# jhidalgocarrio/slam-localization

Hardware: NVIDIA B200
Metric: filter-steps/sec (predict+update) (higher is better)
Workload: dtype f64

## Files before the change

slam-localization_b200/csrc/slb_usckf.cu:

```cuda
#include <cstdlib>

#include "slb_predict12.cuh"
#include "slb_usckf_step.cuh"

namespace slbd {

__global__ void usckf_clone_kernel(slb::FilterArgs a, int mode) {
    const int64_t t = (int64_t)blockIdx.x * blockDim.x + threadIdx.x;
    const int per = 13 + 12 * 12 * 2;
    if (t >= (int64_t)a.B * per) return;
    const int inst = (int)(t / per), e = (int)(t - (int64_t)inst * per);
    double *P = a.P + (size_t)inst * a.pstride, *mu = a.mu + (size_t)inst * a.qstride;
    auto sym = [&](int r, int c) { return r >= c ? P[tri(r, c)] : P[tri(c, r)]; };
    if (e < 13) {
        if (mode == SLB_STATEK_I) mu[13 + e] = mu[26 + e];
        else mu[e] = mu[13 + e];
        return;
    }
    const int q = e - 13, blk = q / 144, rc = q - blk * 144, r = rc / 12, c = rc - r * 12;
    if (mode == SLB_STATEK_I) {
        if (blk == 0) {
            const double v = sym(24 + r, 24 + c);
            if (c <= r) P[tri(12 + r, 12 + c)] = v;
            P[tri(24 + r, 12 + c)] = v;
        } else {
            P[tri(24 + r, c)] = 0.0;
            P[tri(12 + r, c)] = 0.0;
        }
    } else if (blk == 0) {
        const double v = sym(12 + r, 12 + c);
        if (c <= r) P[tri(r, c)] = v;
        P[tri(12 + r, c)] = v;
    }
}

__global__ void usckf_set_measurement_kernel(slb::FilterArgs a, int mode) {
    const int N = 36 + a.nk + a.nl, NP = N * (N + 1) / 2;
    const int nfe = NP - 666;
    const int per = nfe + (mode == SLB_STATEK ? a.nk : a.nl);
    const int64_t t = (int64_t)blockIdx.x * blockDim.x + threadIdx.x;
    if (t >= (int64_t)a.B * per) return;
    const int inst = (int)(t / per), e = (int)(t - (int64_t)inst * per);
    double *P = a.P + (size_t)inst * a.pstride, *mu = a.mu + (size_t)inst * a.qstride;
    const int len = mode == SLB_STATEK ? a.nk : a.nl;
    const int f0 = mode == SLB_STATEK ? 0 : a.nk;
    if (e >= nfe) {
        const int c = e - nfe;
        mu[39 + f0 + c] = a.z[(size_t)inst * len + c];
        return;
    }
    int r = 36;
    while (tri(r + 1, 0) - 666 <= e) ++r;
    const int c = e - (tri(r, 0) - 666);
    const int fr = r - 36, fc = c - 36;
    double v = 0.0;
    if (c >= 36) {
        const bool rin = fr >= f0 && fr < f0 + len, cin = fc >= f0 && fc < f0 + len;
        if (rin && cin) v = a.R[(fr - f0) * len + (fc - f0)];
        else if (!rin && !cin) v = P[tri(r, c)];
    }
    P[tri(r, c)] = v;
}

}

namespace slb {

template <int PM>
static int launch_predict_t(const FilterArgs &a, cudaStream_t s) {
    constexpr int WPB = 8;
    constexpr size_t smem = (size_t)WPB * slbd::PRED_SM * sizeof(double);
    auto kern = slbd::predict12_kernel<PM, WPB, 24, 26, true>;
    SLB_CUDA(cudaFuncSetAttribute(kern, cudaFuncAttributeMaxDynamicSharedMemorySize, (int)smem));
    kern<<<(a.B + WPB - 1) / WPB, WPB * 32, smem, s>>>(a);
    count_launch();
    SLB_CUDA(cudaGetLastError());
    return SLB_OK;
}

#define SLB_USCKF_SHAPES(X) X(3, 0) X(3, 3) X(3, 6) X(3, 9) X(6, 0) X(6, 3) X(6, 6) X(9, 0) X(9, 3)
bool usckf_shape_supported(int nk, int nl) {
#define SLB_USCKF_SHAPE(NK_, NL_) \
    if (nk == NK_ && nl == NL_) return true;
    SLB_USCKF_SHAPES(SLB_USCKF_SHAPE)
#undef SLB_USCKF_SHAPE
    return false;
}

template <int NK, int NL, bool PRED, bool UPD>
static int launch_step_t(const FilterArgs &a, cudaStream_t s) {
    typedef slbd::StepCfg<NK, NL> C;
    constexpr size_t pw = (size_t)C::SM * sizeof(double);
    constexpr size_t SM_BYTES = 228 * 1024, CTA_MAX = 227 * 1024, RSV = 1024;
#ifdef SLB_USCKF_WPB
    constexpr int WPB = SLB_USCKF_WPB;
#else
    constexpr int WPB = 2 * (6 * pw + RSV) <= SM_BYTES ? 6 : 4;
#endif
    constexpr size_t smem = (size_t)WPB * pw;
    constexpr int fit = (int)(SM_BYTES / (smem + RSV));
    constexpr int cap = 12 / WPB < 1 ? 1 : 12 / WPB;
    constexpr int MINB = fit > cap ? cap : fit < 1 ? 1 : fit;
    auto kern = slbd::usckf_step_kernel<SLB_PM_USCKF_TEST, NK, NL, PRED, UPD, WPB, MINB>;
    SLB_CUDA(cudaFuncSetAttribute(kern, cudaFuncAttributeMaxDynamicSharedMemorySize, (int)smem));
    static const int ahead = [] {
        const char *e = getenv("SLB_USCKF_PREFETCH");
        int dev = 0, sms = 148;
        cudaGetDevice(&dev);
        cudaDeviceGetAttribute(&sms, cudaDevAttrMultiProcessorCount, dev);
        return (e ? atoi(e) : 0) * sms * WPB * MINB;
    }();
    FilterArgs b = a;
    b.prefetch = ahead;
    static const size_t pad = [] {
        const char *e = getenv("SLB_USCKF_CTAS");
        const int n = e ? atoi(e) : 0;
        return n == 1 ? (size_t)(200 * 1024) - smem : n == 2 ? (size_t)(110 * 1024) - smem : (size_t)0;
    }();
    if (pad) SLB_CUDA(cudaFuncSetAttribute(kern, cudaFuncAttributeMaxDynamicSharedMemorySize, (int)(smem + pad)));
    kern<<<(a.B + WPB - 1) / WPB, WPB * 32, smem + pad, s>>>(b);
    count_launch();
    SLB_CUDA(cudaGetLastError());
    return SLB_OK;
}

template <int NK, int NL>
static int launch_step_nknl(bool predict, const FilterArgs &a, cudaStream_t s) {
    return predict ? launch_step_t<NK, NL, true, true>(a, s) : launch_step_t<NK, NL, false, true>(a, s);
}

int launch_usckf(int pm, int mm, bool predict, bool update, const FilterArgs &a, cudaStream_t s) {
    if (predict && pm != SLB_PM_USCKF_TEST) return set_error(SLB_ERR_INVALID, "usckf: unsupported process model");
    if (update && mm != SLB_MM_USCKF_VO) return set_error(SLB_ERR_INVALID, "usckf: unsupported measurement model");
    if (predict && !update) return launch_predict_t<SLB_PM_USCKF_TEST>(a, s);
    if (update) {
#define SLB_USCKF_SHAPE(NK_, NL_) \
    if (a.nk == NK_ && a.nl == NL_) return launch_step_nknl<NK_, NL_>(predict, a, s);
        SLB_USCKF_SHAPES(SLB_USCKF_SHAPE)
#undef SLB_USCKF_SHAPE
        return set_error(SLB_ERR_INVALID, "usckf update: (nk, nl) is not one of the built shapes (see slb_usckf_shape_supported)");
    }
    return SLB_OK;
}

int launch_usckf_clone(int mode, const FilterArgs &a, cudaStream_t s) {
    if (mode != SLB_STATEK_I && mode != SLB_STATEK_L) return SLB_OK;
    const int64_t work = (int64_t)a.B * (13 + 288);
    slbd::usckf_clone_kernel<<<(unsigned)((work + 255) / 256), 256, 0, s>>>(a, mode);
    count_launch();
    SLB_CUDA(cudaGetLastError());
    return SLB_OK;
}

int launch_usckf_set_measurement(int mode, const FilterArgs &a, cudaStream_t s) {
    if (mode != SLB_STATEK && mode != SLB_STATEK_L) return SLB_OK;
    const int N = 36 + a.nk + a.nl;
    const int len = mode == SLB_STATEK ? a.nk : a.nl;
    if (len == 0) return SLB_OK;
    const int64_t work = (int64_t)a.B * (N * (N + 1) / 2 - 666 + len);
    slbd::usckf_set_measurement_kernel<<<(unsigned)((work + 255) / 256), 256, 0, s>>>(a, mode);
    count_launch();
    SLB_CUDA(cudaGetLastError());
    return SLB_OK;
}

}
```

slam-localization_b200/csrc/slb_usckf_step.cuh:

```cuda
#pragma once
#include "slb_predict12.cuh"

#ifndef SLB_USCKF_CTA_SYNC
#define SLB_USCKF_CTA_SYNC 0
#endif
#if SLB_USCKF_CTA_SYNC
#define SLB_CTA_SYNC() __syncthreads()
#else
#define SLB_CTA_SYNC() ((void)0)
#endif

namespace slbd {

template <int NK_, int NL_>
struct StepCfg {
    static constexpr int NK = NK_, NL = NL_, NF = NK_ + NL_;
    static constexpr int N = 36 + NK_ + NL_;
    static constexpr int NP = N * (N + 1) / 2;
    static constexpr int PSTR = (NP + 15) / 16 * 16;
    static constexpr int QD = 39 + NK_ + NL_;
    static constexpr int QS = (QD + 1) / 2 * 2;
    static constexpr int NT = (N + 7) / 8;
    static constexpr int NPAD = 8 * NT;
    static constexpr int JM = 36 + NK_;
    static constexpr int NPAN = (JM + 3) / 4;
    static constexpr int NCOL = 4 * NPAN;
    static constexpr int JLAST = (NCOL - 1) >> 3;
    static constexpr int NGRP = (NPAN + 3) / 4;
    static constexpr int PL = 2 * NPAD + 8;
    static constexpr int PS4 = 2 * PL + 2;
    static constexpr int KP = (NK_ + 3) / 4 * 4;
    static constexpr int LF = 4 * PS4;
    static constexpr int LRAW = 2 * PL;
    static constexpr int KK = 2 * NPAD * KP + NPAD;
    static constexpr int SCR0 = (LF + LRAW > KK ? LF + LRAW : KK);
    static constexpr int WGS = 16 * NK_;
    static constexpr int UPD_SCR = SCR0 + WGS + NPAD;
    static constexpr int PRED_SCR = PRED_LS + 28 * PRED_DS + 144 + 12 * PRED_DS + 16 + 16;
    static constexpr int SCR = (UPD_SCR > PRED_SCR ? UPD_SCR : PRED_SCR);
    static constexpr int ZS = (NK_ + 1) / 2 * 2;
    static constexpr int SM = PSTR + QS + SCR + ZS + 2;
    static_assert(NK_ % 3 == 0 && NK_ >= 3, "the VO model moves 3-D features");
    static_assert(N <= 64, "two rows per lane");
    static_assert(SM % 2 == 0 && PSTR % 2 == 0 && QS % 2 == 0, "16-byte alignment of the bulk copies");
};

SLB_DEV void bulk_s2g(void *gdst, const void *ssrc, unsigned bytes) {
    asm volatile("cp.async.bulk.global.shared::cta.bulk_group [%0], [%1], %2;\n cp.async.bulk.commit_group;\n" ::"l"(gdst),
                 "r"(saddr(ssrc)), "r"(bytes)
                 : "memory");
}
SLB_DEV void bulk_prefetch_l2(const void *gsrc, unsigned bytes) {
    asm volatile("cp.async.bulk.prefetch.L2.global [%0], %1;\n" ::"l"(gsrc), "r"(bytes) : "memory");
}
SLB_DEV void bulk_store_wait() { asm volatile("cp.async.bulk.wait_group.read 0;\n" ::: "memory"); }
SLB_DEV void fence_proxy_async() { asm volatile("fence.proxy.async.shared::cta;\n" ::: "memory"); }

template <int M>
SLB_DEV bool sym_inverse(const double *S, double *Si) {
    double L[M * (M + 1) / 2], dd[M], rd[M];
    bool ok = true;
#pragma unroll
    for (int k = 0; k < M; ++k) {
        double d = S[tri(k, k)];
#pragma unroll
        for (int p = 0; p < k; ++p) d = fma(-L[tri(k, p)] * L[tri(k, p)], dd[p], d);
        ok = ok && (d > 0.0);
        dd[k] = d;
        rd[k] = rcp_fast(d);
#pragma unroll
        for (int i = k + 1; i < M; ++i) {
            double s = S[tri(i, k)];
#pragma unroll
            for (int p = 0; p < k; ++p) s = fma(-L[tri(i, p)] * L[tri(k, p)], dd[p], s);
            L[tri(i, k)] = s * rd[k];
        }
    }
    double X[M * (M + 1) / 2];
#pragma unroll
    for (int j = 0; j < M; ++j) {
        X[tri(j, j)] = 1.0;
#pragma unroll
        for (int i = j + 1; i < M; ++i) {
            double s = 0.0;
#pragma unroll
            for (int p = j; p < i; ++p) s = fma(-L[tri(i, p)], X[tri(p, j)], s);
            X[tri(i, j)] = s;
        }
    }
#pragma unroll
    for (int i = 0; i < M; ++i)
#pragma unroll
        for (int j = 0; j <= i; ++j) {
            double s = 0.0;
#pragma unroll
            for (int k = i; k < M; ++k) s = fma(X[tri(k, i)] * rd[k], X[tri(k, j)], s);
            Si[tri(i, j)] = s;
        }
    return ok;
}

template <int NK>
SLB_DEV void vo_model(const double *pk, const double *qk, const double *pi, const double *qi, const double *f, double *z) {
    double dq[4];
    quat_cmul(qi, qk, dq);
#pragma unroll
    for (int c = 0; c < NK; c += 3) {
        double rz[3];
        rotmat_apply(dq, f + c, rz);
        z[c] = rz[0] + (pk[0] - pi[0]);
        z[c + 1] = rz[1] + (pk[1] - pi[1]);
        z[c + 2] = rz[2] + (pk[2] - pi[2]);
    }
}

SLB_DEV void warp_sum12(const double *v, double *out, double *slots, int lane) {
    double a[8], b[4], c[2], d1;
    const bool h16 = lane & 16, h8 = lane & 8, h4 = lane & 4, h2 = lane & 2;
#pragma unroll
    for (int i = 0; i < 8; ++i) {
        const double lo = v[i], hi = i < 4 ? v[8 + i] : 0.0;
        const double r = __shfl_xor_sync(FULL, h16 ? lo : hi, 16);
        a[i] = (h16 ? hi : lo) + r;
    }
#pragma unroll
    for (int i = 0; i < 4; ++i) {
        const double r = __shfl_xor_sync(FULL, h8 ? a[i] : a[4 + i], 8);
        b[i] = (h8 ? a[4 + i] : a[i]) + r;
    }
#pragma unroll
    for (int i = 0; i < 2; ++i) {
        const double r = __shfl_xor_sync(FULL, h4 ? b[i] : b[2 + i], 4);
        c[i] = (h4 ? b[2 + i] : b[i]) + r;
    }
    {
        const double r = __shfl_xor_sync(FULL, h2 ? c[0] : c[1], 2);
        d1 = (h2 ? c[1] : c[0]) + r;
    }
    d1 += __shfl_xor_sync(FULL, d1, 1);
    const int idx = (h16 ? 8 : 0) + (h8 ? 4 : 0) + (h4 ? 2 : 0) + (h2 ? 1 : 0);
    __syncwarp();
    if (!(lane & 1)) slots[idx] = d1;
    __syncwarp();
#pragma unroll
    for (int i = 0; i < 6; ++i) {
        const double2 t = *reinterpret_cast<const double2 *>(slots + 2 * i);
        out[2 * i] = t.x;
        out[2 * i + 1] = t.y;
    }
}

template <class C>
struct UpdState {
    double c0[C::NT][C::JLAST + 1], c1[C::NT][C::JLAST + 1];
    double px0[C::NK], px1[C::NK];
    double esum[C::NK], eep[C::NK * (C::NK + 1) / 2];
    double z0[C::NK];
    bool ok;
};

template <class C, int G>
SLB_DEV void sigma_group(UpdState<C> &s, const double *mus_, const double *Lf, double *Wg, const double *dv, int lane) {
    constexpr int NK = C::NK, PS4 = C::PS4;
    double mus[40 + NK];
    {
        const double2 *m2 = reinterpret_cast<const double2 *>(mus_);
#pragma unroll
        for (int e = 0; e < 4; ++e) { const double2 v = m2[e]; mus[2 * e] = v.x; mus[2 * e + 1] = v.y; }
#pragma unroll
        for (int e = 13; e < 17; ++e) { const double2 v = m2[e]; mus[2 * e] = v.x; mus[2 * e + 1] = v.y; }
#pragma unroll
        for (int c = 0; c < NK; ++c) mus[39 + c] = mus_[39 + c];
    }
    constexpr int col0 = 16 * G;
    constexpr int ncols = C::NCOL - col0 < 16 ? C::NCOL - col0 : 16;
    const bool neg = lane & 1, act = (lane >> 1) < ncols;
    const int jl = act ? lane >> 1 : 0;
    const double rs = rsqrt_fast(dv[col0 + jl]);
    const double sgn = act ? (neg ? -rs : rs) : 0.0;
    const double *col = Lf + (jl >> 2) * PS4 + ((jl & 3) >> 1) * C::PL + (jl & 1);
    auto Lc = [&](int r) -> double { return sgn * col[2 * r]; };
    double xpk[3], xqk[4], xpi[3], xqi[4], xf[NK];
    if (col0 <= 5) {
#pragma unroll
        for (int c = 0; c < 3; ++c) xpk[c] = mus[c] + Lc(c);
        const double v[3] = {Lc(3), Lc(4), Lc(5)};
        const double q[4] = {mus[3], mus[4], mus[5], mus[6]};
        double e[4];
        so3_exp(v, 1.0, e);
        quat_mul(q, e, xqk);
    } else {
#pragma unroll
        for (int c = 0; c < 3; ++c) xpk[c] = mus[c];
#pragma unroll
        for (int c = 0; c < 4; ++c) xqk[c] = mus[3 + c];
    }
    if (col0 <= 29) {
#pragma unroll
        for (int c = 0; c < 3; ++c) xpi[c] = mus[26 + c] + Lc(24 + c);
        const double v[3] = {Lc(27), Lc(28), Lc(29)};
        const double q[4] = {mus[29], mus[30], mus[31], mus[32]};
        double e[4];
        so3_exp(v, 1.0, e);
        quat_mul(q, e, xqi);
    } else {
#pragma unroll
        for (int c = 0; c < 3; ++c) xpi[c] = mus[26 + c];
#pragma unroll
        for (int c = 0; c < 4; ++c) xqi[c] = mus[29 + c];
    }
#pragma unroll
    for (int c = 0; c < NK; ++c) xf[c] = mus[39 + c] + Lc(36 + c);
    double z[NK];
    vo_model<NK>(xpk, xqk, xpi, xqi, xf, z);
    double e[NK];
#pragma unroll
    for (int c = 0; c < NK; ++c) {
        e[c] = act ? z[c] - s.z0[c] : 0.0;
        s.esum[c] += e[c];
        const double zp = __shfl_xor_sync(FULL, z[c], 1);
        if (act && !neg) Wg[c * 16 + jl] = (0.5 * rs) * (z[c] - zp);
    }
#pragma unroll
    for (int r = 0; r < NK; ++r)
#pragma unroll
        for (int c = 0; c <= r; ++c) s.eep[tri(r, c)] = fma(e[r], e[c], s.eep[tri(r, c)]);
    __syncwarp();
    const bool has1 = lane + 32 < C::NPAD;
#pragma unroll
    for (int qq = 0; qq < ncols / 4; ++qq) {
        const double *pa = Lf + qq * PS4 + 2 * lane, *pb = pa + C::PL;
        const double2 x01 = *reinterpret_cast<const double2 *>(pa), x23 = *reinterpret_cast<const double2 *>(pb);
        double2 y01 = make_double2(0.0, 0.0), y23 = y01;
        if (has1) { y01 = *reinterpret_cast<const double2 *>(pa + 64); y23 = *reinterpret_cast<const double2 *>(pb + 64); }
#pragma unroll
        for (int c = 0; c < NK; ++c) {
            const double2 w01 = *reinterpret_cast<const double2 *>(Wg + c * 16 + 4 * qq);
            const double2 w23 = *reinterpret_cast<const double2 *>(Wg + c * 16 + 4 * qq + 2);
            s.px0[c] = fma(x23.y, w23.y, fma(x23.x, w23.x, fma(x01.y, w01.y, fma(x01.x, w01.x, s.px0[c]))));
            s.px1[c] = fma(y23.y, w23.y, fma(y23.x, w23.x, fma(y01.y, w01.y, fma(y01.x, w01.x, s.px1[c]))));
        }
    }
}

template <class C, int P>
struct PanelStep {
    SLB_DEV static void run(UpdState<C> &s, const double *mus, double *Lf, double *Lraw, double *Wg, double *dv, int lane) {
        constexpr int NT = C::NT, JLAST = C::JLAST, PS4 = C::PS4;
        constexpr int K = 4 * P, J0 = K >> 3, H = (K >> 2) & 1, Q = P & 3;
        constexpr int I1 = (K + 4) >> 3;
        const int a_ = lane & 3, b_ = lane >> 2;
        double *Lq = Lf + Q * PS4;
        constexpr int PL = C::PL;
        if ((a_ >> 1) == H) {
#pragma unroll
            for (int I = J0; I < NT; ++I)
                *reinterpret_cast<double2 *>(Lraw + (a_ & 1) * PL + 2 * (8 * I + b_)) = make_double2(s.c0[I][J0], s.c1[I][J0]);
        }
        __syncwarp();
        double m10, m20, m30, m21, m31, m32, r0, r1, r2, r3, d0, d1, d2, d3;
        {
            const double *A = Lraw + 2 * K, *Bp = A + PL;
            const double a00 = A[0];
            const double2 a1 = *reinterpret_cast<const double2 *>(A + 2);
            const double2 a2 = *reinterpret_cast<const double2 *>(A + 4);
            const double a22 = Bp[4];
            const double2 a3 = *reinterpret_cast<const double2 *>(A + 6), a3b = *reinterpret_cast<const double2 *>(Bp + 6);
            d0 = a00;
            r0 = rcp_fast(d0);
            m10 = a1.x * r0; m20 = a2.x * r0; m30 = a3.x * r0;
            d1 = fma(-a1.x, m10, a1.y);
            const double u21 = fma(-a2.x, m10, a2.y), u31 = fma(-a3.x, m10, a3.y);
            r1 = rcp_fast(d1);
            m21 = u21 * r1; m31 = u31 * r1;
            d2 = fma(-u21, m21, fma(-a2.x, m20, a22));
            const double u32 = fma(-u31, m21, fma(-a3.x, m20, a3b.x));
            r2 = rcp_fast(d2);
            m32 = u32 * r2;
            d3 = fma(-u32, m32, fma(-u31, m31, fma(-a3.x, m30, a3b.y)));
            r3 = rcp_fast(d3);
            s.ok = s.ok && (d0 > 0.0) && (d1 > 0.0) && (d2 > 0.0) && (d3 > 0.0);
        }
        if (lane == 0) {
            *reinterpret_cast<double2 *>(dv + K) = make_double2(d0, d1);
            *reinterpret_cast<double2 *>(dv + K + 2) = make_double2(d2, d3);
        }
        auto finish = [&](int i, bool have) {
            const double2 x01 = *reinterpret_cast<const double2 *>(Lraw + 2 * i);
            const double2 x23 = *reinterpret_cast<const double2 *>(Lraw + PL + 2 * i);
            const double u0 = x01.x;
            const double u1 = fma(-u0, m10, x01.y);
            const double u2 = fma(-u1, m21, fma(-u0, m20, x23.x));
            const double u3 = fma(-u2, m32, fma(-u1, m31, fma(-u0, m30, x23.y)));
            double2 u01, u23;
            u01.x = i >= K ? u0 : 0.0;
            u01.y = i >= K + 1 ? u1 : 0.0;
            u23.x = i >= K + 2 ? u2 : 0.0;
            u23.y = i >= K + 3 ? u3 : 0.0;
            if (have) {
                *reinterpret_cast<double2 *>(Lq + 2 * i) = u01;
                *reinterpret_cast<double2 *>(Lq + PL + 2 * i) = u23;
            }
        };
        if (K < 32) {
            finish(lane, true);
        } else {
            *reinterpret_cast<double2 *>(Lq + 2 * lane) = make_double2(0.0, 0.0);
            *reinterpret_cast<double2 *>(Lq + PL + 2 * lane) = make_double2(0.0, 0.0);
        }
        if (C::NPAD > 32) finish(lane + 32 < C::NPAD ? lane + 32 : lane, lane + 32 < C::NPAD);
        __syncwarp();
        if (I1 <= JLAST) {
            double f[NT];
            const double *fp = Lq + (a_ >> 1) * PL + (a_ & 1) + 2 * b_;
#pragma unroll
            for (int I = I1; I < NT; ++I) f[I] = fp[16 * I];
            const double rlo = (a_ & 1) ? r1 : r0, rhi = (a_ & 1) ? r3 : r2;
            const double nr = -((a_ & 2) ? rhi : rlo);
#pragma unroll
            for (int J = I1; J <= JLAST; ++J) {
                const double g = f[J] * nr;
#pragma unroll
                for (int I = J; I < NT; ++I) dmma884(s.c0[I][J], s.c1[I][J], f[I], g);
            }
        }
        if (Q == 3 || P == C::NPAN - 1) {
            sigma_group<C, (P >> 2)>(s, mus, Lf, Wg, dv, lane);
            SLB_CTA_SYNC();
        }
        PanelStep<C, P + 1>::run(s, mus, Lf, Lraw, Wg, dv, lane);
    }
};
template <class C>
struct PanelStep<C, C::NPAN> {
    SLB_DEV static void run(UpdState<C> &, const double *, double *, double *, double *, double *, int) {}
};

template <int NK, int NL>
SLB_DEV int usckf_update_smem(double *Ps, double *mus, double *scr, const double *zs, const slb::FilterArgs &a, int lane,
                              bool &dirty) {
    typedef StepCfg<NK, NL> C;
    constexpr int N = C::N, NT = C::NT, NPAD = C::NPAD, JLAST = C::JLAST, KP = C::KP;
    const int a_ = lane & 3, b_ = lane >> 2;
    double *Lf = scr, *Lraw = scr + C::LF, *Ks = scr, *Cs = scr + NPAD * KP, *Wg = scr + C::SCR0, *dv = Wg + C::WGS,
           *dl = Cs + NPAD * KP;
    UpdState<C> s;
    s.ok = true;
    auto elem = [&](int i, int j) -> double {
        if (i >= N || j >= N) return i == j ? 1.0 : 0.0;
        return i >= j ? Ps[tri(i, j)] : Ps[tri(j, i)];
    };
#pragma unroll
    for (int I = 0; I < NT; ++I)
#pragma unroll
        for (int J = 0; J <= JLAST; ++J)
            if (J <= I) {
                const int i = 8 * I + b_, j = 8 * J + 2 * a_;
                s.c0[I][J] = elem(i, j);
                s.c1[I][J] = elem(i, j + 1);
            }
#pragma unroll
    for (int c = 0; c < NK; ++c) s.px0[c] = s.px1[c] = s.esum[c] = 0.0;
#pragma unroll
    for (int e = 0; e < NK * (NK + 1) / 2; ++e) s.eep[e] = 0.0;
    {
        double pk[3], qk[4], pi[3], qi[4], ft[NK];
#pragma unroll
        for (int c = 0; c < 3; ++c) { pk[c] = mus[c]; pi[c] = mus[26 + c]; }
#pragma unroll
        for (int c = 0; c < 4; ++c) { qk[c] = mus[3 + c]; qi[c] = mus[29 + c]; }
#pragma unroll
        for (int c = 0; c < NK; ++c) ft[c] = mus[39 + c];
        vo_model<NK>(pk, qk, pi, qi, ft, s.z0);
    }
    PanelStep<C, 0>::run(s, mus, Lf, Lraw, Wg, dv, lane);
    if (!s.ok) return SLB_ST_CHOL_FAIL;

    constexpr double NS = (double)(2 * N + 1);
    double ebar[NK], S[NK * (NK + 1) / 2];
    if (NK == 3) {
        double v[12], o[12];
#pragma unroll
        for (int c = 0; c < 3; ++c) v[c] = s.esum[c];
#pragma unroll
        for (int e = 0; e < 6; ++e) v[3 + e] = s.eep[e];
        v[9] = v[10] = v[11] = 0.0;
        warp_sum12(v, o, dv, lane);
#pragma unroll
        for (int c = 0; c < 3; ++c) ebar[c] = o[c] * (1.0 / NS);
#pragma unroll
        for (int r = 0; r < NK; ++r)
#pragma unroll
            for (int c = 0; c <= r; ++c)
                S[tri(r, c)] = 0.5 * fma(-NS * ebar[r], ebar[c], o[3 + tri(r, c)]) + __ldg(a.R + r * NK + c);
    } else {
#pragma unroll
        for (int c = 0; c < NK; ++c) ebar[c] = warp_sum(s.esum[c]) * (1.0 / NS);
#pragma unroll
        for (int r = 0; r < NK; ++r)
#pragma unroll
            for (int c = 0; c <= r; ++c)
                S[tri(r, c)] = 0.5 * fma(-NS * ebar[r], ebar[c], warp_sum(s.eep[tri(r, c)])) + __ldg(a.R + r * NK + c);
    }
    double Si[NK * (NK + 1) / 2];
    const bool sok = sym_inverse<NK>(S, Si);
    auto SiAt = [&](int r, int c) { return r >= c ? Si[tri(r, c)] : Si[tri(c, r)]; };
    asm volatile("cp.async.wait_group 0;\n" ::: "memory");
    __syncwarp();
    double nu[NK], sn[NK], m2 = 0.0;
#pragma unroll
    for (int c = 0; c < NK; ++c) nu[c] = zs[c] - (s.z0[c] + ebar[c]);
#pragma unroll
    for (int r = 0; r < NK; ++r) {
        double t = 0.0;
#pragma unroll
        for (int c = 0; c < NK; ++c) t = fma(SiAt(r, c), nu[c], t);
        sn[r] = t;
        m2 = fma(nu[r], t, m2);
    }
    if (!sok) return SLB_ST_CHOL_FAIL;
    if (!chi2_accept(m2, a.gate)) return SLB_ST_GATE_REJECT;
    auto finish_row = [&](const double *px, int i) {
        double dsum = 0.0;
#pragma unroll
        for (int c = 0; c < KP; ++c) {
            double k = 0.0;
            if (c < NK) {
#pragma unroll
                for (int p = 0; p < NK; ++p) k = fma(px[p], SiAt(p, c), k);
                dsum = fma(px[c], sn[c], dsum);
            }
            Ks[i * KP + c] = k;
            Cs[i * KP + c] = c < NK ? -px[c] : 0.0;
        }
        dl[i] = dsum;
    };
    finish_row(s.px0, lane);
    if (lane + 32 < NPAD) finish_row(s.px1, lane + 32);
    __syncwarp();
    dirty = true;
    bool finite = true;
    if (lane < 12) {
        const int mbw = lane & 3;
        const int mqo = 13 * (lane >> 2) + (mbw == 0 ? 0 : mbw == 1 ? 3 : mbw == 2 ? 7 : 10);
        const double v[3] = {dl[3 * lane], dl[3 * lane + 1], dl[3 * lane + 2]};
        if (mbw == 1) {
            const double q[4] = {mus[mqo], mus[mqo + 1], mus[mqo + 2], mus[mqo + 3]};
            double e[4], o[4];
            so3_exp(v, 1.0, e);
            quat_mul(q, e, o);
#pragma unroll
            for (int c = 0; c < 4; ++c) { mus[mqo + c] = o[c]; finite = finite && isfinite(o[c]); }
        } else {
#pragma unroll
            for (int c = 0; c < 3; ++c) {
                const double o = mus[mqo + c] + v[c];
                mus[mqo + c] = o;
                finite = finite && isfinite(o);
            }
        }
    }
    for (int f = lane; f < NK + NL; f += 32) {
        const double o = mus[39 + f] + dl[36 + f];
        mus[39 + f] = o;
        finite = finite && isfinite(o);
    }
    {
        double fa[NT][KP / 4], fb[NT][KP / 4];
#pragma unroll
        for (int I = 0; I < NT; ++I)
#pragma unroll
            for (int kk = 0; kk < KP / 4; ++kk) {
                fa[I][kk] = Cs[(8 * I + b_) * KP + 4 * kk + a_];
                fb[I][kk] = Ks[(8 * I + b_) * KP + 4 * kk + a_];
            }
#pragma unroll
        for (int I = 0; I < NT; ++I)
#pragma unroll
            for (int J = 0; J <= I; ++J) {
                const int i = 8 * I + b_, j = 8 * J + 2 * a_;
                const bool w0 = i < N && j <= i, w1 = i < N && j + 1 <= i;
                double p0 = w0 ? Ps[tri(i, j)] : 0.0, p1 = w1 ? Ps[tri(i, j + 1)] : 0.0;
#pragma unroll
                for (int kk = 0; kk < KP / 4; ++kk) dmma884(p0, p1, fa[I][kk], fb[J][kk]);
                if (w0) Ps[tri(i, j)] = p0;
                if (w1) Ps[tri(i, j + 1)] = p1;
            }
    }
    return __all_sync(FULL, finite) ? 0 : SLB_ST_NONFINITE;
}

template <int PM, int NF>
SLB_DEV int usckf_predict_smem(double *Ps, double *mus, double *scr, const double *u, double dt, const double *Qg, int lane,
                               bool &dirty) {
    typedef LayState12 L;
    typedef CycCfg<12> C;
    constexpr int ROW0 = 24, MU0 = 26;
    double *Ls = scr, *D = Ls + PRED_LS, *W = D + 28 * PRED_DS, *Fk = W + 144, *rsd = Fk + 12 * PRED_DS, *slots = rsd + 16;
    auto PR = [&](int r, int c) -> double & { return Ps[tri(ROW0 + r, c)]; };
    auto PF = [&](int fr, int c) -> double & { return Ps[tri(36 + fr, 24 + c)]; };
    const int a_ = lane & 3, b_ = lane >> 2;
    double mu[13];
#pragma unroll
    for (int c = 0; c < 13; ++c) mu[c] = mus[MU0 + c];
    ProcessModel<PM> f;
    f.prepare(u, dt);
    double T[C::RT][C::CT];
#pragma unroll
    for (int r = 0; r < C::RT; ++r)
#pragma unroll
        for (int c = 0; c < C::CT; ++c)
            if (C::exists(r, c)) {
                const int i = a_ + 4 * r, j = b_ + 8 * c;
                T[r][c] = (i < 12 && j <= i) ? PR(i, ROW0 + j) : 0.0;
            }
    bool ok = true;
    {
        const double x0 = __shfl_sync(FULL, T[0][0], 0);
        CholStep<C, 0>::run(T, Ls, a_, b_, ok, x0, -rcp_fast(x0));
    }
    if (!ok) return SLB_ST_CHOL_FAIL;
    __syncwarp();
    if (lane < 12) {
        double sq_, rs_;
        sqrt_rsqrt(Ls[C::cb(lane)], sq_, rs_);
        rsd[lane] = rs_;
    }
    __syncwarp();
    const bool act = lane < 25;
    const int j = lane >= 1 ? (lane - 1) >> 1 : 0, jc = j < 12 ? j : 11;
    double Y[13];
    {
        const double sgn = (lane & 1) ? rsd[jc] : -rsd[jc];
        const int cj = C::cb(jc) - jc;
        double d[12], X[13];
#pragma unroll
        for (int r = 0; r < 12; ++r) d[r] = (act && lane >= 1 && r >= jc) ? sgn * Ls[cj + r] : 0.0;
        boxplus<L>(mu, d, 1.0, X);
        f.apply(X, Y);
    }
    double ref[13];
#pragma unroll
    for (int c = 0; c < 13; ++c) ref[c] = bcast(Y[c], 0);
    int it = 0;
    double nrm2;
    do {
        double dd[12], md[12], nr[13];
        boxminus<L>(Y, ref, dd);
#pragma unroll
        for (int r = 0; r < 12; ++r) dd[r] = act ? dd[r] : 0.0;
        warp_sum12(dd, md, slots, lane);
        nrm2 = 0.0;
#pragma unroll
        for (int r = 0; r < 12; ++r) {
            md[r] *= (1.0 / 25.0);
            nrm2 += md[r] * md[r];
        }
        boxplus<L>(ref, md, 1.0, nr);
#pragma unroll
        for (int c = 0; c < 13; ++c) ref[c] = nr[c];
    } while (sqrt(nrm2) > 1e-6 && ++it < 10000);
    int st = (it >= 10000) ? SLB_ST_MEAN_NOCONV : 0;
    {
        double dY[12];
        boxminus<L>(Y, ref, dY);
        if (lane < 28) {
#pragma unroll
            for (int r = 0; r < 12; r += 2)
                *reinterpret_cast<double2 *>(D + lane * PRED_DS + r) = act ? make_double2(dY[r], dY[r + 1]) : make_double2(0.0, 0.0);
        }
    }
    __syncwarp();
    dirty = true;
    {
        double c00[2] = {0.0, 0.0}, c10[2] = {0.0, 0.0}, c11[2] = {0.0, 0.0};
        const double *p0 = D + a_ * PRED_DS + b_, *p1 = p0 + 8;
#pragma unroll
        for (int k0 = 0; k0 < 28; k0 += 4) {
            const double f0 = p0[k0 * PRED_DS], f1 = p1[k0 * PRED_DS];
            dmma884(c00[0], c00[1], f0, f0);
            dmma884(c10[0], c10[1], f1, f0);
            dmma884(c11[0], c11[1], f1, f1);
        }
        for (int e = lane; e < 144; e += 32) {
            const int jj = e / 12, c = e - jj * 12;
            W[e] = 0.5 * (D[(1 + 2 * jj) * PRED_DS + c] - D[(2 + 2 * jj) * PRED_DS + c]);
        }
        __syncwarp();
        auto put = [&](int r, int c, double v) {
            if (r < 12 && c <= r) PR(r, ROW0 + c) = 0.5 * v + __ldg(Qg + r * 12 + c);
        };
        const int r = b_, c = 2 * a_;
        put(r, c, c00[0]); put(r, c + 1, c00[1]);
        put(8 + r, c, c10[0]); put(8 + r, c + 1, c10[1]);
        put(8 + r, 8 + c, c11[0]); put(8 + r, 8 + c + 1, c11[1]);
    }
    if (lane < 12) {
        double x[12];
#pragma unroll
        for (int r = 11; r >= 0; --r) {
            double sacc = 0.0;
#pragma unroll
            for (int p = r + 1; p < 12; ++p) sacc = fma(Ls[C::cb(r) - r + p], x[p], sacc);
            const double rs = rsd[r];
            x[r] = (W[r * 12 + lane] - rs * sacc) * rs;
        }
#pragma unroll
        for (int r = 0; r < 12; ++r) Fk[lane * PRED_DS + r] = x[r];
    }
    __syncwarp();
    double oc[2][3][2];
    {
        const int r0 = min(b_, 11), r1 = min(8 + b_, 11);
#pragma unroll
        for (int I = 0; I < 2; ++I)
#pragma unroll
            for (int J = 0; J < 3; ++J) oc[I][J][0] = oc[I][J][1] = 0.0;
#pragma unroll
        for (int k0 = 0; k0 < 12; k0 += 4) {
            const double fa0 = Fk[r0 * PRED_DS + k0 + a_], fa1 = Fk[r1 * PRED_DS + k0 + a_];
#pragma unroll
            for (int J = 0; J < 3; ++J) {
                const double bv = PR(k0 + a_, 8 * J + b_);
                dmma884(oc[0][J][0], oc[0][J][1], fa0, bv);
                dmma884(oc[1][J][0], oc[1][J][1], fa1, bv);
            }
        }
    }
    constexpr int NFT = (NF + 7) / 8;
    double of[NFT > 0 ? NFT : 1][2][2];
    {
        const int c0 = min(b_, 11), c1 = min(8 + b_, 11);
#pragma unroll
        for (int I = 0; I < NFT; ++I) {
            of[I][0][0] = of[I][0][1] = of[I][1][0] = of[I][1][1] = 0.0;
            const int fr = min(8 * I + b_, NF - 1);
#pragma unroll
            for (int k0 = 0; k0 < 12; k0 += 4) {
                const double av = PF(fr, k0 + a_);
                dmma884(of[I][0][0], of[I][0][1], av, Fk[c0 * PRED_DS + k0 + a_]);
                dmma884(of[I][1][0], of[I][1][1], av, Fk[c1 * PRED_DS + k0 + a_]);
            }
        }
    }
    __syncwarp();
#pragma unroll
    for (int I = 0; I < 2; ++I)
#pragma unroll
        for (int J = 0; J < 3; ++J) {
            const int r = 8 * I + b_, c = 8 * J + 2 * a_;
            if (r < 12) { PR(r, c) = oc[I][J][0]; PR(r, c + 1) = oc[I][J][1]; }
        }
#pragma unroll
    for (int I = 0; I < NFT; ++I) {
#pragma unroll
        for (int J = 0; J < 2; ++J) {
            const int fr = 8 * I + b_, c = 8 * J + 2 * a_;
            if (fr < NF && c < 12) { PF(fr, c) = of[I][J][0]; PF(fr, c + 1) = of[I][J][1]; }
        }
    }
    bool finite = true;
#pragma unroll
    for (int c = 0; c < 13; ++c) {
        finite = finite && isfinite(ref[c]);
        if (lane == c) mus[MU0 + c] = ref[c];
    }
    if (!finite) st |= SLB_ST_NONFINITE;
    __syncwarp();
    return st;
}

template <int PM, int NK, int NL, bool PRED, bool UPD, int WPB, int MINB>
__global__ void __launch_bounds__(WPB * 32, MINB) usckf_step_kernel(slb::FilterArgs a) {
    typedef StepCfg<NK, NL> C;
    extern __shared__ __align__(128) double smem[];
    const int lane = threadIdx.x & 31, w = threadIdx.x >> 5;
    const int inst = blockIdx.x * WPB + w;
    if (inst >= a.B) return;
    double *Ps = smem + (size_t)w * C::SM, *mus = Ps + C::PSTR, *scr = mus + C::QS, *zs = scr + C::SCR;
    uint64_t *bar = reinterpret_cast<uint64_t *>(zs + C::ZS);
    double *Pg = a.P + (size_t)inst * a.pstride;
    double *mug = a.mu + (size_t)inst * a.qstride;
    if (lane == 0) {
        mbar_init(bar, 1);
        mbar_expect_tx(bar, (C::PSTR + C::QS) * 8);
        bulk_g2s(Ps, Pg, C::PSTR * 8, bar);
        bulk_g2s(mus, mug, C::QS * 8, bar);
        if (a.prefetch > 0 && inst + a.prefetch < a.B) bulk_prefetch_l2(Pg + (size_t)a.prefetch * a.pstride, C::PSTR * 8);
    }
    if (UPD && lane < NK) {
        asm volatile("cp.async.ca.shared.global [%0], [%1], 8;\n cp.async.commit_group;\n" ::"r"(saddr(zs + lane)),
                     "l"(a.z + (size_t)inst * NK + lane)
                     : "memory");
    }
    double u[ProcessModel<PM>::NU];
    if (PRED) {
#pragma unroll
        for (int c = 0; c < ProcessModel<PM>::NU; ++c) u[c] = a.u[(size_t)inst * ProcessModel<PM>::NU + c];
    }
    __syncwarp();
    mbar_wait(bar, 0);
    SLB_CTA_SYNC();
    int st = 0;
    bool dirty = false;
    if (PRED) st |= usckf_predict_smem<PM, NK + NL>(Ps, mus, scr, u, a.dt, a.Q, lane, dirty);
    if (PRED) SLB_CTA_SYNC();
    if (UPD) st |= usckf_update_smem<NK, NL>(Ps, mus, scr, zs, a, lane, dirty);
    asm volatile("cp.async.wait_group 0;\n" ::: "memory");
    if (dirty) {
        fence_proxy_async();
        __syncwarp();
        if (lane == 0) bulk_s2g(Pg, Ps, C::PSTR * 8);
        for (int e = lane; e < C::QD; e += 32) mug[e] = mus[e];
    }
    if (a.mu_out) {
        __syncwarp();
        for (int e = lane; e < a.out_len; e += 32) a.mu_out[(size_t)inst * a.out_len + e] = mus[a.out_off + e];
    }
    if (st && lane == 0) a.status[inst] |= st;
    if (dirty && lane == 0) bulk_store_wait();
}

}
```

Measured before the change: 92.15 million.

## Accumulate UKF cross-covariance with DMMA tiles and trim panel finish work

```diff
diff --git a/profiles/sass_smem.py b/profiles/sass_smem.py
--- /dev/null
+++ b/profiles/sass_smem.py
@@ -0,0 +1,43 @@
+import os
+import re
+import subprocess
+import sys
+from collections import Counter
+
+ROOT = os.path.dirname(os.path.dirname(os.path.abspath(__file__)))
+LIB = sys.argv[1] if len(sys.argv) > 1 else os.path.join(ROOT, "slam-localization_b200", "csrc", "libslb.so")
+KERNEL = "usckf_step_kernel<4, 3, 9, true, true"
+WIDTH = {"": 32, "U8": 8, "S8": 8, "U16": 16, "S16": 16, "64": 64, "128": 128}
+
+sass = subprocess.run(["cuobjdump", "-sass", LIB], capture_output=True, text=True, check=True).stdout
+funcs, cur = {}, None
+for line in sass.splitlines():
+    m = re.search(r"Function : (\S+)", line)
+    if m:
+        cur = m.group(1)
+        funcs[cur] = []
+    elif cur is not None:
+        funcs[cur].append(line)
+names = list(funcs)
+demangled = subprocess.run(["c++filt"], input="\n".join(names), capture_output=True, text=True).stdout.splitlines()
+hits = [n for n, d in zip(names, demangled) if KERNEL in d]
+assert len(hits) == 1, "expected one %s in %s" % (KERNEL, LIB)
+count = Counter()
+for line in funcs[hits[0]]:
+    m = re.match(r"\s+/\*[0-9a-f]+\*/\s+(?:@!?U?P\w+\s+)?(LDS|STS|SHFL)((?:\.\w+)*)\s", line)
+    if not m:
+        continue
+    mods = [x for x in m.group(2).split(".") if x]
+    if m.group(1) == "SHFL":
+        count[("SHFL", 32)] += 1
+    else:
+        count[(m.group(1), max([WIDTH[x] for x in mods if x in WIDTH] or [32]))] += 1
+print("# cuobjdump -sass %s (sm_100a): %s, predict+update> -- static counts" % (os.path.relpath(LIB, ROOT), KERNEL))
+print("%-6s %5s %6s %11s" % ("op", "bits", "count", "wavefronts"))
+tot = Counter()
+for (op, w), n in sorted(count.items()):
+    wf = n * max(1, w // 32)
+    tot[op] += wf
+    tot["all"] += wf
+    print("%-6s %5d %6d %11d" % (op, w, n, wf))
+print("wavefront-weighted: LDS %d, STS %d, SHFL %d, total %d" % (tot["LDS"], tot["STS"], tot["SHFL"], tot["all"]))
diff --git a/profiles/usckf_phases.py b/profiles/usckf_phases.py
--- /dev/null
+++ b/profiles/usckf_phases.py
@@ -0,0 +1,40 @@
+import ctypes
+import os
+import sys
+
+import numpy as np
+
+ROOT = os.path.dirname(os.path.dirname(os.path.abspath(__file__)))
+sys.path.insert(0, ROOT)
+import torch
+import bench
+from slam_localization_b200 import engine
+
+NAMES = ["record wait (TMA bulk load)",
+         "predict: factorisation (CholStep 12x12)", "predict: sigma points + process model", "predict: manifold mean",
+         "predict: deviations, D^T D + W", "predict: Fk solve", "predict: cross-covariances + mean out",
+         "update: tile fill + Z0 = h(mu)",
+         "update: panels 0-3", "update: sigma pass 0", "update: panels 4-7", "update: sigma pass 1",
+         "update: panels 8-9", "update: sigma pass 2",
+         "update: sums / S^-1 / gain", "update: mean [+]", "update: Pk -= covXZ K^T", "store"]
+CTAS, WARPS, SLOTS = 16, 16, 24
+
+assert os.environ.get("SLB_LIB"), "set SLB_LIB to the instrumented libslb_phases.so"
+wl = bench.UsckfWorkload(0)
+wl.setup_gpu(engine, torch)
+for k in range(4):
+    wl.step(k)
+torch.cuda.synchronize()
+lib = ctypes.CDLL(os.environ["SLB_LIB"])
+out = np.zeros(CTAS * WARPS * SLOTS, dtype=np.int64)
+assert lib.slb_debug_usckf_phases(out.ctypes.data_as(ctypes.c_void_p)) == 0
+t = out.reshape(CTAS * WARPS, SLOTS)[:, :len(NAMES) + 1]
+t = t[(t > 0).all(axis=1)]
+d = np.diff(t, axis=1)
+tot = np.median(t[:, -1] - t[:, 0])
+print("usckf_step_kernel<3,9> fused step, %d instances, %d stamped warps: median %d cycles per instance (warp)"
+      % (wl.B, len(t), tot))
+for k, name in enumerate(NAMES):
+    m = np.median(d[:, k])
+    print("  %-44s %7d  (%4.1f %%)   p10 %7d  p90 %7d" % (name, m, 100.0 * m / tot, np.percentile(d[:, k], 10),
+                                                        np.percentile(d[:, k], 90)))
diff --git a/slam-localization_b200/csrc/slb_usckf.cu b/slam-localization_b200/csrc/slb_usckf.cu
--- a/slam-localization_b200/csrc/slb_usckf.cu
+++ b/slam-localization_b200/csrc/slb_usckf.cu
@@ -165,3 +165,9 @@
 }
 
 }
+
+#ifdef SLB_USCKF_PHASES
+extern "C" int slb_debug_usckf_phases(long long *out) {
+    return (int)cudaMemcpyFromSymbol(out, slbd::us_phase_dbg, sizeof(slbd::us_phase_dbg));
+}
+#endif
diff --git a/slam-localization_b200/csrc/slb_usckf_step.cuh b/slam-localization_b200/csrc/slb_usckf_step.cuh
--- a/slam-localization_b200/csrc/slb_usckf_step.cuh
+++ b/slam-localization_b200/csrc/slb_usckf_step.cuh
@@ -11,6 +11,19 @@
 #endif
 
 namespace slbd {
+
+#ifdef SLB_USCKF_PHASES
+constexpr int US_PH_CTAS = 16, US_PH_WARPS = 16, US_PH_SLOTS = 24;
+__device__ long long us_phase_dbg[US_PH_CTAS * US_PH_WARPS * US_PH_SLOTS];
+#define US_PH(slot)                                                                                             \
+    do {                                                                                                        \
+        const unsigned c_ = blockIdx.x - gridDim.x / 2;                                                         \
+        if (c_ < US_PH_CTAS && (threadIdx.x & 31) == 0)                                                         \
+            us_phase_dbg[(c_ * US_PH_WARPS + (threadIdx.x >> 5)) * US_PH_SLOTS + (slot)] = clock64();           \
+    } while (0)
+#else
+#define US_PH(slot) do { } while (0)
+#endif
 
 template <int NK_, int NL_>
 struct StepCfg {
@@ -30,11 +43,13 @@
     static constexpr int PL = 2 * NPAD + 8;
     static constexpr int PS4 = 2 * PL + 2;
     static constexpr int KP = (NK_ + 3) / 4 * 4;
+    static constexpr int NKT = (NK_ + 7) / 8;
     static constexpr int LF = 4 * PS4;
     static constexpr int LRAW = 2 * PL;
     static constexpr int KK = 2 * NPAD * KP + NPAD;
     static constexpr int SCR0 = (LF + LRAW > KK ? LF + LRAW : KK);
-    static constexpr int WGS = 16 * NK_;
+    static constexpr int WST = 20;
+    static constexpr int WGS = WST * NK_;
     static constexpr int UPD_SCR = SCR0 + WGS + NPAD;
     static constexpr int PRED_SCR = PRED_LS + 28 * PRED_DS + 144 + 12 * PRED_DS + 16 + 16;
     static constexpr int SCR = (UPD_SCR > PRED_SCR ? UPD_SCR : PRED_SCR);
@@ -153,7 +168,7 @@
 template <class C>
 struct UpdState {
     double c0[C::NT][C::JLAST + 1], c1[C::NT][C::JLAST + 1];
-    double px0[C::NK], px1[C::NK];
+    double cx[C::NT][C::NKT][2];
     double esum[C::NK], eep[C::NK * (C::NK + 1) / 2];
     double z0[C::NK];
     bool ok;
@@ -179,7 +194,7 @@
     const double rs = rsqrt_fast(dv[col0 + jl]);
     const double sgn = act ? (neg ? -rs : rs) : 0.0;
     const double *col = Lf + (jl >> 2) * PS4 + ((jl & 3) >> 1) * C::PL + (jl & 1);
-    auto Lc = [&](int r) -> double { return sgn * col[2 * r]; };
+    auto Lc = [&](int r) -> double { return r >= col0 + 15 || r >= col0 + jl ? sgn * col[2 * r] : 0.0; };
     double xpk[3], xqk[4], xpi[3], xqi[4], xf[NK];
     if (col0 <= 5) {
 #pragma unroll
@@ -219,26 +234,30 @@
         e[c] = act ? z[c] - s.z0[c] : 0.0;
         s.esum[c] += e[c];
         const double zp = __shfl_xor_sync(FULL, z[c], 1);
-        if (act && !neg) Wg[c * 16 + jl] = (0.5 * rs) * (z[c] - zp);
+        if (act && !neg) Wg[c * C::WST + jl] = (0.5 * rs) * (z[c] - zp);
     }
 #pragma unroll
     for (int r = 0; r < NK; ++r)
 #pragma unroll
         for (int c = 0; c <= r; ++c) s.eep[tri(r, c)] = fma(e[r], e[c], s.eep[tri(r, c)]);
     __syncwarp();
-    const bool has1 = lane + 32 < C::NPAD;
+    const int a_ = lane & 3, b_ = lane >> 2;
 #pragma unroll
     for (int qq = 0; qq < ncols / 4; ++qq) {
-        const double *pa = Lf + qq * PS4 + 2 * lane, *pb = pa + C::PL;
-        const double2 x01 = *reinterpret_cast<const double2 *>(pa), x23 = *reinterpret_cast<const double2 *>(pb);
-        double2 y01 = make_double2(0.0, 0.0), y23 = y01;
-        if (has1) { y01 = *reinterpret_cast<const double2 *>(pa + 64); y23 = *reinterpret_cast<const double2 *>(pb + 64); }
-#pragma unroll
-        for (int c = 0; c < NK; ++c) {
-            const double2 w01 = *reinterpret_cast<const double2 *>(Wg + c * 16 + 4 * qq);
-            const double2 w23 = *reinterpret_cast<const double2 *>(Wg + c * 16 + 4 * qq + 2);
-            s.px0[c] = fma(x23.y, w23.y, fma(x23.x, w23.x, fma(x01.y, w01.y, fma(x01.x, w01.x, s.px0[c]))));
-            s.px1[c] = fma(y23.y, w23.y, fma(y23.x, w23.x, fma(y01.y, w01.y, fma(y01.x, w01.x, s.px1[c]))));
+        const int K = col0 + 4 * qq;
+        double w[C::NKT];
+#pragma unroll
+        for (int T = 0; T < C::NKT; ++T) {
+            const int n = 8 * T + b_;
+            const double v = Wg[(n < NK ? n : NK - 1) * C::WST + 4 * qq + a_];
+            w[T] = n < NK ? v : 0.0;
+        }
+        const double *fp = Lf + qq * PS4 + (a_ >> 1) * C::PL + (a_ & 1) + 2 * b_;
+#pragma unroll
+        for (int I = K >> 3; I < C::NT; ++I) {
+            const double f = 8 * I >= K || 8 * I + b_ >= K ? fp[16 * I] : 0.0;
+#pragma unroll
+            for (int T = 0; T < C::NKT; ++T) dmma884(s.cx[I][T][0], s.cx[I][T][1], f, w[T]);
         }
     }
 }
@@ -285,7 +304,7 @@
             *reinterpret_cast<double2 *>(dv + K) = make_double2(d0, d1);
             *reinterpret_cast<double2 *>(dv + K + 2) = make_double2(d2, d3);
         }
-        auto finish = [&](int i, bool have) {
+        auto finish = [&](int i) {
             const double2 x01 = *reinterpret_cast<const double2 *>(Lraw + 2 * i);
             const double2 x23 = *reinterpret_cast<const double2 *>(Lraw + PL + 2 * i);
             const double u0 = x01.x;
@@ -293,22 +312,16 @@
             const double u2 = fma(-u1, m21, fma(-u0, m20, x23.x));
             const double u3 = fma(-u2, m32, fma(-u1, m31, fma(-u0, m30, x23.y)));
             double2 u01, u23;
-            u01.x = i >= K ? u0 : 0.0;
+            u01.x = u0;
             u01.y = i >= K + 1 ? u1 : 0.0;
             u23.x = i >= K + 2 ? u2 : 0.0;
             u23.y = i >= K + 3 ? u3 : 0.0;
-            if (have) {
-                *reinterpret_cast<double2 *>(Lq + 2 * i) = u01;
-                *reinterpret_cast<double2 *>(Lq + PL + 2 * i) = u23;
-            }
+            *reinterpret_cast<double2 *>(Lq + 2 * i) = u01;
+            *reinterpret_cast<double2 *>(Lq + PL + 2 * i) = u23;
         };
-        if (K < 32) {
-            finish(lane, true);
-        } else {
-            *reinterpret_cast<double2 *>(Lq + 2 * lane) = make_double2(0.0, 0.0);
-            *reinterpret_cast<double2 *>(Lq + PL + 2 * lane) = make_double2(0.0, 0.0);
-        }
-        if (C::NPAD > 32) finish(lane + 32 < C::NPAD ? lane + 32 : lane, lane + 32 < C::NPAD);
+        constexpr int R = C::NPAD - K;
+        if (R >= 32 || lane < R) finish(K + lane);
+        if (R > 32 && lane < R - 32) finish(K + 32 + lane);
         __syncwarp();
         if (I1 <= JLAST) {
             double f[NT];
@@ -325,7 +338,9 @@
             }
         }
         if (Q == 3 || P == C::NPAN - 1) {
+            US_PH(9 + 2 * (P >> 2));
             sigma_group<C, (P >> 2)>(s, mus, Lf, Wg, dv, lane);
+            US_PH(10 + 2 * (P >> 2));
             SLB_CTA_SYNC();
         }
         PanelStep<C, P + 1>::run(s, mus, Lf, Lraw, Wg, dv, lane);
@@ -360,7 +375,11 @@
                 s.c1[I][J] = elem(i, j + 1);
             }
 #pragma unroll
-    for (int c = 0; c < NK; ++c) s.px0[c] = s.px1[c] = s.esum[c] = 0.0;
+    for (int c = 0; c < NK; ++c) s.esum[c] = 0.0;
+#pragma unroll
+    for (int I = 0; I < NT; ++I)
+#pragma unroll
+        for (int T = 0; T < C::NKT; ++T) s.cx[I][T][0] = s.cx[I][T][1] = 0.0;
 #pragma unroll
     for (int e = 0; e < NK * (NK + 1) / 2; ++e) s.eep[e] = 0.0;
     {
@@ -373,6 +392,7 @@
         for (int c = 0; c < NK; ++c) ft[c] = mus[39 + c];
         vo_model<NK>(pk, qk, pi, qi, ft, s.z0);
     }
+    US_PH(8);
     PanelStep<C, 0>::run(s, mus, Lf, Lraw, Wg, dv, lane);
     if (!s.ok) return SLB_ST_CHOL_FAIL;
 
@@ -420,7 +440,21 @@
     }
     if (!sok) return SLB_ST_CHOL_FAIL;
     if (!chi2_accept(m2, a.gate)) return SLB_ST_GATE_REJECT;
-    auto finish_row = [&](const double *px, int i) {
+#pragma unroll
+    for (int I = 0; I < NT; ++I)
+#pragma unroll
+        for (int T = 0; T < C::NKT; ++T)
+            if (8 * T + 2 * a_ < KP)
+                *reinterpret_cast<double2 *>(Cs + (8 * I + b_) * KP + 8 * T + 2 * a_) = make_double2(-s.cx[I][T][0], -s.cx[I][T][1]);
+    __syncwarp();
+    auto finish_row = [&](int i) {
+        double px[KP];
+#pragma unroll
+        for (int c = 0; c < KP; c += 2) {
+            const double2 v = *reinterpret_cast<const double2 *>(Cs + i * KP + c);
+            px[c] = -v.x;
+            px[c + 1] = -v.y;
+        }
         double dsum = 0.0;
 #pragma unroll
         for (int c = 0; c < KP; ++c) {
@@ -431,13 +465,13 @@
                 dsum = fma(px[c], sn[c], dsum);
             }
             Ks[i * KP + c] = k;
-            Cs[i * KP + c] = c < NK ? -px[c] : 0.0;
         }
         dl[i] = dsum;
     };
-    finish_row(s.px0, lane);
-    if (lane + 32 < NPAD) finish_row(s.px1, lane + 32);
-    __syncwarp();
+    finish_row(lane);
+    if (lane + 32 < NPAD) finish_row(lane + 32);
+    __syncwarp();
+    US_PH(15);
     dirty = true;
     bool finite = true;
     if (lane < 12) {
@@ -465,6 +499,7 @@
         mus[39 + f] = o;
         finite = finite && isfinite(o);
     }
+    US_PH(16);
     {
         double fa[NT][KP / 4], fb[NT][KP / 4];
 #pragma unroll
@@ -487,6 +522,7 @@
                 if (w1) Ps[tri(i, j + 1)] = p1;
             }
     }
+    US_PH(17);
     return __all_sync(FULL, finite) ? 0 : SLB_ST_NONFINITE;
 }
 
@@ -527,6 +563,7 @@
         rsd[lane] = rs_;
     }
     __syncwarp();
+    US_PH(2);
     const bool act = lane < 25;
     const int j = lane >= 1 ? (lane - 1) >> 1 : 0, jc = j < 12 ? j : 11;
     double Y[13];
@@ -539,6 +576,7 @@
         boxplus<L>(mu, d, 1.0, X);
         f.apply(X, Y);
     }
+    US_PH(3);
     double ref[13];
 #pragma unroll
     for (int c = 0; c < 13; ++c) ref[c] = bcast(Y[c], 0);
@@ -561,6 +599,7 @@
         for (int c = 0; c < 13; ++c) ref[c] = nr[c];
     } while (sqrt(nrm2) > 1e-6 && ++it < 10000);
     int st = (it >= 10000) ? SLB_ST_MEAN_NOCONV : 0;
+    US_PH(4);
     {
         double dY[12];
         boxminus<L>(Y, ref, dY);
@@ -595,20 +634,23 @@
         put(8 + r, c, c10[0]); put(8 + r, c + 1, c10[1]);
         put(8 + r, 8 + c, c11[0]); put(8 + r, 8 + c + 1, c11[1]);
     }
+    US_PH(5);
     if (lane < 12) {
-        double x[12];
+        double x[12], sacc[12];
+#pragma unroll
+        for (int r = 0; r < 12; ++r) sacc[r] = 0.0;
 #pragma unroll
         for (int r = 11; r >= 0; --r) {
-            double sacc = 0.0;
-#pragma unroll
-            for (int p = r + 1; p < 12; ++p) sacc = fma(Ls[C::cb(r) - r + p], x[p], sacc);
             const double rs = rsd[r];
-            x[r] = (W[r * 12 + lane] - rs * sacc) * rs;
+            x[r] = (W[r * 12 + lane] - rs * sacc[r]) * rs;
+#pragma unroll
+            for (int q = 0; q < r; ++q) sacc[q] = fma(Ls[C::cb(q) - q + r], x[r], sacc[q]);
         }
 #pragma unroll
         for (int r = 0; r < 12; ++r) Fk[lane * PRED_DS + r] = x[r];
     }
     __syncwarp();
+    US_PH(6);
     double oc[2][3][2];
     {
         const int r0 = min(b_, 11), r1 = min(8 + b_, 11);
@@ -667,6 +709,7 @@
     }
     if (!finite) st |= SLB_ST_NONFINITE;
     __syncwarp();
+    US_PH(7);
     return st;
 }
 
@@ -681,6 +724,7 @@
     uint64_t *bar = reinterpret_cast<uint64_t *>(zs + C::ZS);
     double *Pg = a.P + (size_t)inst * a.pstride;
     double *mug = a.mu + (size_t)inst * a.qstride;
+    US_PH(0);
     if (lane == 0) {
         mbar_init(bar, 1);
         mbar_expect_tx(bar, (C::PSTR + C::QS) * 8);
@@ -700,6 +744,7 @@
     }
     __syncwarp();
     mbar_wait(bar, 0);
+    US_PH(1);
     SLB_CTA_SYNC();
     int st = 0;
     bool dirty = false;
@@ -719,6 +764,7 @@
     }
     if (st && lane == 0) a.status[inst] |= st;
     if (dirty && lane == 0) bulk_store_wait();
-}
-
-}
+    US_PH(18);
+}
+
+}
```

Result: faster. 93.74 million (median of 6 runs) (+1.7%).
